# clearmatics/zecale

Measured on AMD Instinct MI355X. Metric: G1-MSM Mscalar/s (BW6_761, 2^20 terms per GPU), higher is better.
Workload: dtype u32; 1 GPU; BASELINE configs[1]: single MI355X G1_BW6_761 Pippenger MSM, 2^20 random scalars/points; terms_per_gpu=1048576, scalars=uniform in [0, r), Montgomery residues as libff holds them, parallelism=point-partitioned x1, RCCL all-gather of 288-byte partial sums

## Files before the change

include/zkhip.h:

```cpp
#ifndef ZKHIP_H
#define ZKHIP_H
#include <stddef.h>
#include <stdint.h>

#ifdef __cplusplus
extern "C" {
#endif

#define ZKHIP_OK 0
#define ZKHIP_ERR_ARG (-1)
#define ZKHIP_ERR_NO_DEVICE (-2)
#define ZKHIP_ERR_HIP (-3)
#define ZKHIP_ERR_STATE (-4)
#define ZKHIP_ERR_NO_TICKET (-5)

typedef struct zkhip_bases zkhip_bases;

int zkhip_init(int device);
int zkhip_set_device(int device);
int zkhip_get_device(void);
int zkhip_device_count(void);
int zkhip_device_memory(size_t* free_bytes, size_t* total_bytes);
void zkhip_shutdown(void);
const char* zkhip_strerror(int code);
// ... 198 lines not shown

typedef struct zkhip_keypair zkhip_keypair;
int zkhip_groth16_setup(const zkhip_r1cs_desc* cs, const uint64_t tau[6], const uint64_t alpha[6], const uint64_t beta[6],
                        const uint64_t delta[6], zkhip_keypair** out);
int zkhip_groth16_setup_ex(const zkhip_r1cs_desc* cs, const uint64_t tau[6], const uint64_t alpha[6], const uint64_t beta[6],
                           const uint64_t delta[6], size_t domain_size, zkhip_keypair** out);
int zkhip_groth16_setup_slice(const zkhip_r1cs_desc* cs, const uint64_t tau[6], const uint64_t alpha[6], const uint64_t beta[6],
                              const uint64_t delta[6], size_t domain_size, int parts, int part, const zkhip_key_opts* opts,
                              zkhip_crs** slice_out, size_t ranges[6], zkhip_keypair** vk_out);
int zkhip_keypair_crs_desc(const zkhip_keypair* kp, zkhip_crs_desc* out);
size_t zkhip_keypair_vk(const zkhip_keypair* kp, uint64_t alpha_g1[24], uint64_t beta_g2[24], uint64_t delta_g2[24],
                        const uint64_t** abc);
int zkhip_keypair_write(const zkhip_keypair* kp, const char* path);
int zkhip_keypair_read(const char* path, zkhip_keypair** out);
void zkhip_keypair_free(zkhip_keypair* kp);

float zkhip_last_accumulate_ms(void);
int zkhip_last_accumulate_entries(uint64_t* out);
int zkhip_last_accumulate_interval(float out_ms[2]);
int zkhip_reset_time_base(void);
int zkhip_measure_fq_mul_rate(double* fq_mul_per_s);
int zkhip_measure_ntt(unsigned log_d, int dir, int coset, int batch, int reps, double* ms_per_transform);
int zkhip_internal_field_selftest(int field, const uint32_t* limbs_in, size_t n, uint32_t* limbs_out);
int zkhip_internal_fq6_selftest(int op, const uint64_t* a, const uint64_t* b, size_t n, uint64_t* out);
int zkhip_internal_pairing_product(int route, const uint64_t* g1, const uint64_t* g2, size_t pairs_per_product, size_t count, uint64_t* out);
int zkhip_internal_tail_selftest(const uint64_t g1[24], const uint64_t g2[24], const uint64_t small_order_g1[24], int rounds);
typedef struct zkhip_witness_program {
  const uint8_t* code;
  const int32_t* a;
  const int32_t* b;
  size_t n_pos;
  const uint32_t* level_start;
  size_t n_levels;
  uint32_t chain_start;
  const int32_t* out_ref;
  size_t n_vars;
  const uint64_t* consts;
  size_t n_consts;
  size_t n_inputs;
} zkhip_witness_program;
int zkhip_internal_witness_run_program(const zkhip_witness_program* p, const uint64_t* inputs, size_t batches, int witnesses_per_workgroup,
                                       unsigned segment_chunks, uint64_t* z_out, uint32_t* flags_out);
int zkhip_internal_witness_run_program_wide(const zkhip_witness_program* p, const uint64_t* inputs, size_t batches, int witnesses_per_workgroup,
                                            unsigned segment_chunks, int waves, uint64_t* z_out, uint32_t* flags_out);
int zkhip_internal_pipeline_witness_sizing(size_t value_bytes, size_t mem_total, size_t wit_batch, int workers, size_t out[2]);
int zkhip_internal_witness_tape(zkhip_aggregator* a, zkhip_witness_program* out);
// ... 39 lines not shown
```

zecale_amd/csrc/msm.h:

```cpp
#pragma once
#include <hip/hip_runtime.h>
#include <stddef.h>
#include <stdint.h>

#include "../../include/zkhip.h"

namespace zkhip {

struct AffPacked;
struct EdwPacked;

#define MSM_MAX_AFF_LEVELS 4
#define MSM_MAX_JOBS 5
struct MsmJob {
  const AffPacked* bases;
  const uint8_t* inf_flags;
  const uint64_t* scalars;
  size_t n;
  int scalars_mode;
  size_t table_stride;
  size_t n_finite;
  const EdwPacked* edw = nullptr;
};
static inline size_t msm_job_terms(const MsmJob& j) { return (j.n_finite && j.n_finite < j.n) ? j.n_finite : j.n; }
// ... 1 lines not shown
#define ZK_PRIO_BOARD_WORDS (8 * 8 * 2 * 16 * 4 * 16)
struct MsmCtx {
  bool planned;
  int c, W, L, logL;
  int Wd;
  int merged;
  int K;
  uint16_t win_off[96];
  uint8_t win_bits[96];
  size_t B, max_n;
  size_t total_terms;
  int one_stream;
  uint32_t quad_below;
  uint32_t S, T, slot_stride;
  hipStream_t stream, stream2;
  hipEvent_t ev, ev2, ev_acc0, ev_acc1, ev_done;
  hipEvent_t acc_gate;
  uint32_t sort_LB, sort_NP, sort_bins, sort_tile;
  uint32_t* hist;
  uint2* pairs;
  size_t hist_len;
  uint32_t *counts, *offsets, *block_tot, *entries;
  uint32_t* goff;
  uint2* fix_list;
  uint2* fix_short;
  uint32_t *buckets, *segS[2], *segR, *sumR[2], *Rlevels, *colS[2], *hilo;
  uint64_t *win_abi, *win_host;
  int aff_levels;
  int aff_forced;
  uint32_t aff_m, aff_lanes;
  uint32_t *lcnt[MSM_MAX_AFF_LEVELS], *loff[MSM_MAX_AFF_LEVELS];
  AffPacked* pbuf[2];
  uint32_t* aff_scratch;
  size_t m_acc_max;
  float last_accumulate_ms;
  size_t last_hist_m;
  uint32_t acc_gen;
  float last_acc_begin_ms, last_acc_end_ms;
  uint64_t* dbg_times;
  uint32_t* prio_board;
  uint32_t prio_seq;
  uint32_t last_S, last_T;
  int last_tight;
  bool pending;
  size_t pending_n;
  bool win_edw;
  char errbuf[256];
};

void msm_force_aff_levels(int levels);
int msm_forced_aff_levels();
int msm_plan_init(MsmCtx* ctx, size_t max_n, int c, int merged, int K, size_t total_terms = 0, hipStream_t* adopt = nullptr);
hipEvent_t msm_time_base();
int msm_time_base_reset();
void msm_plan_free(MsmCtx* ctx);
int msm_bases_convert(const uint64_t* d_bases_abi, size_t n, AffPacked* d_out, uint8_t* d_inf_flags, char* errbuf, size_t errlen);
int msm_launch(MsmCtx* ctx, const AffPacked* d_bases, const uint8_t* d_inf_flags, const uint64_t* d_scalars, size_t n,
               int scalars_montgomery, size_t table_stride, const EdwPacked* edw = nullptr);
int msm_finish(MsmCtx* ctx, uint64_t out_jac[36]);
int msm_last_entries(MsmCtx* ctx, uint64_t* out);
int msm_launch_multi(MsmCtx* ctx, int K, const MsmJob* jobs);
int msm_finish_multi(MsmCtx* ctx, int K, uint64_t* out_jac);
static inline int msm_table_levels(int c, int naf = 0) { return naf ? 378 : (378 + c - 1) / c; }
int msm_table_build(AffPacked* d_table, uint8_t* d_tinf, size_t n, int c, int naf, char* errbuf, size_t errlen);
int msm_table_edw(const AffPacked* d_bases, const uint8_t* d_inf, size_t n, int c, EdwPacked** d_out, char* errbuf, size_t errlen);
static inline const EdwPacked* msm_edw_at(const EdwPacked* t, size_t i) {
  return t ? reinterpret_cast<const EdwPacked*>(reinterpret_cast<const char*>(t) + i * 288) : nullptr;
}

int msm_field_selftest(int field, const uint32_t* in_host, size_t n, uint32_t* out_host, char* errbuf, size_t errlen);
int msm_measure_fqmul_rate(double* fq_mul_per_s, char* errbuf, size_t errlen);

int fixed_base_mul(const uint64_t base_aff[24], const uint64_t* d_scalars, size_t n, int montgomery, uint64_t* d_out,
                   char* errbuf, size_t errlen);
// ... 3 lines not shown
```

zecale_amd/csrc/msm.hip:

```cpp
#include <hip/hip_runtime.h>
#include <stdint.h>
#include <stdio.h>
#include <stdlib.h>
#include <string.h>
#include <mutex>
#include <vector>

#include "ec_affine.cuh"
#include "ec_edw.cuh"
#include "host_field.hpp"
#include "msm.h"
#include "wait.h"


namespace zkhip {


__global__ void __launch_bounds__(256) k_bases_to_dev(const uint64_t* __restrict__ in, AffPacked* __restrict__ out,
                                                       uint8_t* __restrict__ inf_flags , size_t n) {
  size_t i = (size_t)blockIdx.x * blockDim.x + threadIdx.x;
  if (i >= n) return;
  uint64_t x[12], y[12];
  uint64_t nz = 0;
#pragma unroll
// ... 488 lines not shown
    const AffPacked* p = (dense ? bp.p[0] : base_of<NJ>(bp, b >> bshift)) + (e & 0x7fffffffu);
    const bool neg = (e >> 31) != 0;
    k++;
    if (dense && p->x[23] == ZK_AFF_INF_WORD) continue;
    if (madd_lds_regy(acc, xs, zz, zzz, ty, p, neg)) inf = fp_is_zero_2p(lds_ld(zz));
  }
  if (board_mine && (threadIdx.x & 63u) == 0) __hip_atomic_store(board_mine, (prio_tag << 16) | 0xffffu, __ATOMIC_RELAXED, __HIP_MEMORY_SCOPE_AGENT);
  if (!inf) {
    ZK_CLOSE_RUN(acc, xs, zz, zzz, ty);
  }
  if (dbg_times && (threadIdx.x & 63u) == 0) {
    const uint32_t wave = t >> 6;
    dbg_times[4 * wave] = dbg_t0; dbg_times[4 * wave + 1] = wall_clock64();
    dbg_times[4 * wave + 2] = __builtin_amdgcn_s_getreg((31 << 11) | 4);
    dbg_times[4 * wave + 3] = __builtin_amdgcn_s_getreg((31 << 11) | 20);
  }
}
template <int NJ>
__global__ void __launch_bounds__(256, 2) k_accumulate(ZK_ACC_PARAMS) {
  accumulate_impl<NJ, false>(bp, bshift, entries, offsets, counts, goff, nb, S_host, tight, T, slots, stride, fix_cnt, fix_short, fix_long,
                             dbg_times, prio_mode, prio_board, prio_tag);
}
__global__ void __launch_bounds__(256, 2) k_accumulate_edw(ZK_ACC_PARAMS) {
  accumulate_impl<1, true>(bp, bshift, entries, offsets, counts, goff, nb, S_host, tight, T, slots, stride, fix_cnt, fix_short, fix_long,
                           dbg_times, prio_mode, prio_board, prio_tag);
}

__global__ void __launch_bounds__(256) k_table_edw(const AffPacked* __restrict__ tab, const uint8_t* __restrict__ tinf, EdwPacked* __restrict__ out,
                                                   size_t total, uint32_t* __restrict__ bad) {
  const size_t i = (size_t)blockIdx.x * blockDim.x + threadIdx.x;
  if (i >= total) return;
  if (tinf[i]) {
    uint32_t* w = reinterpret_cast<uint32_t*>(out + i);
#pragma unroll
    for (int k = 0; k < 72; k++) w[k] = 0u;
    return;
  }
  const AffPacked* p = tab + i;
  if (!edw_from_affine(aff_ld_x(p), aff_ld_y(p, false), out + i)) atomicAdd(bad, 1u);
}

__global__ void __launch_bounds__(256) k_half_counts(const uint32_t* __restrict__ in_cnt, uint32_t* __restrict__ out_cnt, size_t nb) {
  size_t i = (size_t)blockIdx.x * blockDim.x + threadIdx.x;
  if (i < nb) out_cnt[i] = (in_cnt[i] + 1) >> 1;
}

struct LevelArgs {
  BasePtrs bp;
// ... 204 lines not shown
    for (uint32_t i = blockIdx.x * per + (QUAD ? threadIdx.x >> 2 : threadIdx.x); i < n; i += short_blocks * per) {
      const uint2 w = list_short[i];
      const XyzzRef dst = make_slot_ref(slots, stride, nb + w.x);
      for (uint32_t j = 1; j < w.y; j++) pt_add<QUAD, EDW>(dst, make_slot_ref(slots, stride, nb + w.x + j), q, sc);
    }
    return;
  }
  const uint32_t n = cnt[1], quad = threadIdx.x >> 2;
  for (uint32_t i = blockIdx.x - short_blocks; i < n; i += gridDim.x - short_blocks) {
    const uint2 w = list_long[i];
#pragma unroll 1
    for (uint32_t d = 1; d <= w.y - w.x; d <<= 1) {
      for (uint64_t t = (uint64_t)w.x + (uint64_t)quad * 2 * d; t + d <= w.y; t += (uint64_t)64 * 2 * d)
        pt_add<true, EDW>(make_slot_ref(slots, stride, nb + (uint32_t)t), make_slot_ref(slots, stride, nb + (uint32_t)t + d), q, sc);
      __threadfence_block();
      __syncthreads();
    }
  }
}
template <bool QUAD> __global__ void __launch_bounds__(256, 2) k_fixup_fold(ZK_FOLD_PARAMS) {
  fixup_fold_impl<QUAD, false>(cnt, list_short, list_long, short_blocks, nb, slots, stride);
}
template <bool QUAD> __global__ void __launch_bounds__(256, 2) k_fixup_fold_edw(ZK_FOLD_PARAMS) {
  fixup_fold_impl<QUAD, true>(cnt, list_short, list_long, short_blocks, nb, slots, stride);
}

#define ZK_FIXUP_PARAMS                                                                                                             \
  const uint32_t* __restrict__ offsets, const uint32_t* __restrict__ counts, const uint32_t* __restrict__ goff, uint32_t nb, uint32_t S_host, \
      int tight, uint32_t T, uint32_t* __restrict__ slots, uint32_t stride, uint32_t wf
template <bool EDW>
__device__ __forceinline__ void fixup_impl(ZK_FIXUP_PARAMS) {
  __shared__ uint32_t lds_zz[27 * ZK_LDS_STRIDE], lds_zzz[27 * ZK_LDS_STRIDE], lds_x[24 * ZK_LDS_STRIDE];
  uint32_t t = blockIdx.x * blockDim.x + threadIdx.x;
  const uint32_t M = offsets[nb - 1] + counts[nb - 1];
  const uint32_t A = slice_weight(goff[nb], T, S_host, tight);
  if (t >= T) return;
  uint32_t b0_, b1_;
  const uint32_t pos0 = slice_pos(goff, offsets, counts, nb, M, (uint64_t)t * A, &b0_, wf);
  if (pos0 >= M) return;
  const uint32_t pos1 = slice_pos(goff, offsets, counts, nb, M, (uint64_t)(t + 1) * A, &b1_, wf);
  uint32_t b = bucket_of(offsets, nb, pos1 - 1);
  uint32_t bend = offsets[b] + counts[b];
  if (bend <= pos1 || offsets[b] < pos0) return;
  const XyzzRef dst = make_slot_ref(slots, stride, b), pl = make_slot_ref(slots, stride, nb + T + t), pf = make_slot_ref(slots, stride, nb + t + 1);
  const bool l_inf = mem_is_inf(pl), f_inf = mem_is_inf(pf);
  if (l_inf || f_inf) {
    if (l_inf && f_inf) mem_set_inf(dst);
    else mem_copy(dst, l_inf ? pf : pl);
    return;
  }
  uint32_t* zz = lds_zz + threadIdx.x;
  uint32_t* zzz = lds_zzz + threadIdx.x;
  uint32_t* xs = lds_x + threadIdx.x;
  lds_st_packed(xs, mem_ld(pl, CX));
  Fq ty = mem_ld(pl, CY);
  lds_st(zz, mem_ld(pl, CZZ));
  lds_st(zzz, mem_ld(pl, CZZZ));
  if (pt_add_lds<EDW>(dst, xs, zz, zzz, ty, pf)) { mem_set_inf(dst); return; }
  mem_st(dst, CX, lds_ld_packed(xs)); mem_st(dst, CY, ty); mem_st(dst, CZZ, lds_ld(zz)); mem_st(dst, CZZZ, lds_ld(zzz));
}
__global__ void __launch_bounds__(256, 2) k_fixup(ZK_FIXUP_PARAMS) { fixup_impl<false>(offsets, counts, goff, nb, S_host, tight, T, slots, stride, wf); }
__global__ void __launch_bounds__(256, 2) k_fixup_edw(ZK_FIXUP_PARAMS) { fixup_impl<true>(offsets, counts, goff, nb, S_host, tight, T, slots, stride, wf); }

#define ZK_SEG_PARAMS uint32_t* __restrict__ in, size_t n_in, uint32_t in_stride, int L, int o, uint32_t* __restrict__ outS, uint32_t* __restrict__ outR
template <bool QUAD, bool EDW>
__device__ __forceinline__ void seg_impl(ZK_SEG_PARAMS) {
  ADD_SCRATCH_DECL(QUAD || EDW);
  size_t n_out = n_in / L;
  size_t gt = (size_t)blockIdx.x * blockDim.x + threadIdx.x, t = QUAD ? gt >> 2 : gt;
  const uint32_t q = (uint32_t)(gt & 3);
  if (t >= n_out) return;
  XyzzRef run = make_ref(outS, (uint32_t)n_out, (uint32_t)t), acc = make_ref(outR, (uint32_t)n_out, (uint32_t)t);
  pt_set_inf<QUAD>(run, q);
  pt_set_inf<QUAD>(acc, q);
  for (int u = L - 1; u >= 0; u--) {
    XyzzRef it = make_ref(in, in_stride, (uint32_t)(t * L + u));
    pt_add<QUAD, EDW>(run, it, q, sc);
    if (u + o > 0) pt_add<QUAD, EDW>(acc, run, q, sc);
  }
}
template <bool QUAD> __global__ void __launch_bounds__(256, 2) k_seg(ZK_SEG_PARAMS) { seg_impl<QUAD, false>(in, n_in, in_stride, L, o, outS, outR); }
template <bool QUAD> __global__ void __launch_bounds__(256, 2) k_seg_edw(ZK_SEG_PARAMS) { seg_impl<QUAD, true>(in, n_in, in_stride, L, o, outS, outR); }

#define ZK_SUM_PARAMS                                                                                       \
  uint32_t* __restrict__ in, size_t n_in, uint32_t in_stride, int L, uint32_t row_len, uint32_t* __restrict__ out, \
// ... 403 lines not shown
    const char* e = getenv("ZKHIP_SLICE_TARGET");
    v = e ? (size_t)atoi(e) : 80;
    if (v < 8 || v > 4096) v = 80;
  }
  return v;
}

static int env_int(const char* name, int dflt, int lo, int hi) {
  const char* e = getenv(name);
  if (!e) return dflt;
  int v = atoi(e);
  return (v < lo || v > hi) ? dflt : v;
}
static size_t level_bound(size_t m, size_t nb) { return (m + (m < nb ? m : nb)) / 2; }
static int g_aff_forced = -2;
void msm_force_aff_levels(int levels) { g_aff_forced = levels < -1 ? -1 : (levels > MSM_MAX_AFF_LEVELS ? MSM_MAX_AFF_LEVELS : levels); }
int msm_forced_aff_levels() { return g_aff_forced == -2 ? env_int("ZKHIP_AFF_LEVELS", -1, 0, MSM_MAX_AFF_LEVELS) : g_aff_forced; }
static int choose_aff_levels(size_t m_entries, size_t nb) {
  (void)m_entries; (void)nb;
  int forced = msm_forced_aff_levels();
  return forced >= 0 ? forced : 0;
}

static hipEvent_t g_time_base[64];
static bool g_time_base_made[64];
static uint32_t g_time_base_gen[64];
static std::mutex g_time_base_mu;
static hipEvent_t time_base_locked(int dev, bool renew) {
  if (!g_time_base_made[dev] && hipEventCreate(&g_time_base[dev]) != hipSuccess) return nullptr;
  if (!g_time_base_made[dev] || renew) {
    if (hipEventRecord(g_time_base[dev], 0) != hipSuccess || hipEventSynchronize(g_time_base[dev]) != hipSuccess) {
      if (!g_time_base_made[dev]) (void)hipEventDestroy(g_time_base[dev]);
      return nullptr;
    }
    g_time_base_made[dev] = true;
  }
  return g_time_base[dev];
}
hipEvent_t msm_time_base() {
  int dev = 0;
  if (hipGetDevice(&dev) != hipSuccess || dev < 0 || dev >= 64) dev = 0;
  std::lock_guard<std::mutex> lk(g_time_base_mu);
  return time_base_locked(dev, false);
}
int msm_time_base_reset() {
  int dev = 0;
// ... 84 lines not shown
  HIP_TRY(hipEventCreateWithFlags(&ctx->ev_done, hipEventBlockingSync | hipEventDisableTiming));
  if ((size_t)ctx->Wd * max_n >= ((size_t)1 << 31)) return ZKHIP_ERR_ARG;
  if ((size_t)ctx->Wd * total_terms >= ((size_t)1 << 32)) return ZKHIP_ERR_ARG;
  {
    uint32_t LB = (uint32_t)(c - 1 < 10 ? c - 1 : 10);
    const size_t want_parts = (size_t)env_int("ZKHIP_SORT_PARTS", 1024, 64, 8192);
    while (LB > 6 && (nb >> LB) < want_parts && (ctx->B >> (LB - 1)) * (merged ? 1 : (size_t)ctx->Wd) <= 4096) LB--;
    ctx->sort_LB = LB;
    ctx->sort_NP = (uint32_t)(ctx->B >> LB);
    ctx->sort_bins = merged ? ctx->sort_NP : ctx->sort_NP * (uint32_t)ctx->Wd;
    if ((size_t)ctx->sort_bins * 8 > 60 * 1024) return ZKHIP_ERR_ARG;
    uint32_t tile = (uint32_t)env_int("ZKHIP_SORT_TILE", 1024, 256, 16384) & ~255u;
    while ((max_n + tile - 1) / tile > 1024) tile *= 2;
    ctx->sort_tile = tile;
    const size_t nbx = (max_n + tile - 1) / tile;
    ctx->hist_len = (nb >> LB) * (nbx ? nbx : 1) + 1;
  }
  HIP_TRY(hipMalloc(&ctx->hist, ctx->hist_len * 4));
  HIP_TRY(hipMalloc(&ctx->pairs, ((size_t)ctx->Wd * total_terms + 1) * sizeof(uint2)));
  HIP_TRY(hipMalloc(&ctx->counts, nb * 4));
  HIP_TRY(hipMalloc(&ctx->offsets, nb * 4));
  HIP_TRY(hipMalloc(&ctx->goff, (nb + 1) * 4));
  if ((size_t)ctx->Wd * total_terms * ZK_W_NEXT >= ((size_t)1 << 32)) return ZKHIP_ERR_ARG;
  HIP_TRY(hipMalloc(&ctx->block_tot, ((nb > ctx->hist_len ? nb : ctx->hist_len) / 1024 + 2) * 4));
  HIP_TRY(hipMalloc(&ctx->entries, ((size_t)ctx->Wd * total_terms + 1) * 4));
  {
    size_t m = (size_t)ctx->Wd * total_terms;
    ctx->aff_levels = choose_aff_levels(m, nb);
    ctx->aff_forced = msm_forced_aff_levels();
    ctx->aff_m = (uint32_t)env_int("ZKHIP_AFF_M", 64, 4, 512);
    ctx->aff_lanes = 1u << 18;
    const size_t m_cap = (size_t)ctx->aff_m * 3 / 2;
    while ((size_t)ctx->aff_lanes * m_cap * 108 >= ((size_t)1 << 32)) ctx->aff_lanes >>= 1;
    size_t bound[MSM_MAX_AFF_LEVELS + 1];
    bound[0] = m;
    for (int l = 0; l < ctx->aff_levels; l++) {
      bound[l + 1] = level_bound(bound[l], nb);
      HIP_TRY(hipMalloc(&ctx->lcnt[l], nb * 4));
      HIP_TRY(hipMalloc(&ctx->loff[l], nb * 4));
    }
    if (ctx->aff_levels > 0) {
      HIP_TRY(hipMalloc(&ctx->pbuf[0], (bound[1] + 1) * sizeof(AffPacked)));
      if (ctx->aff_levels > 1) HIP_TRY(hipMalloc(&ctx->pbuf[1], (bound[2] + 1) * sizeof(AffPacked)));
      size_t lanes = (bound[1] + ctx->aff_m - 1) / ctx->aff_m;
      if (lanes < ctx->aff_lanes) ctx->aff_lanes = (uint32_t)((lanes + 255) & ~(size_t)255);
      HIP_TRY(hipMalloc(&ctx->aff_scratch, (size_t)ctx->aff_lanes * m_cap * 108));
    }
// ... 20 lines not shown
  ctx->prio_seq = 0;
  HIP_TRY(hipMalloc(&ctx->fix_list, ((size_t)ctx->T / 5 + 2) * sizeof(uint2)));
  HIP_TRY(hipMalloc(&ctx->fix_short, ((size_t)ctx->T / 2 + 2) * sizeof(uint2)));
  HIP_TRY(hipMalloc(&ctx->segS[0], (nb / 2 + 1) * 108 * 4));
  HIP_TRY(hipMalloc(&ctx->segS[1], (nb / 2 + 1) * 108 * 4));
  HIP_TRY(hipMalloc(&ctx->segR, (nb / 2 + 64 * (size_t)ctx->W) * 108 * 4));
  HIP_TRY(hipMalloc(&ctx->sumR[0], (nb / ctx->L / ctx->L + 4 * ctx->W + 1) * 108 * 4));
  HIP_TRY(hipMalloc(&ctx->sumR[1], (nb / ctx->L / ctx->L + 4 * ctx->W + 1) * 108 * 4));
  HIP_TRY(hipMalloc(&ctx->Rlevels, (size_t)32 * 2 * ctx->W * 108 * 4));
  HIP_TRY(hipMalloc(&ctx->colS[0], (nb / 2 + 1) * 108 * 4));
  HIP_TRY(hipMalloc(&ctx->colS[1], (nb / 2 + 1) * 108 * 4));
  HIP_TRY(hipMalloc(&ctx->hilo, ((size_t)2 * ctx->W * ((size_t)1 << ((c - 1 + 1) / 2)) + 8) * 108 * 4));
  HIP_TRY(hipMalloc(&ctx->win_abi, (size_t)ctx->W * 48 * 8 * 2));
  HIP_TRY(hipHostMalloc(&ctx->win_host, (size_t)ctx->W * 48 * 8 * 2));
  ctx->planned = true;
  return ZKHIP_OK;
}

void msm_plan_free(MsmCtx* ctx) {
  void* ptrs[] = {ctx->hist, ctx->pairs, ctx->counts, ctx->offsets, ctx->block_tot, ctx->entries, ctx->buckets,
                  ctx->segS[0], ctx->segS[1], ctx->segR, ctx->sumR[0], ctx->sumR[1], ctx->Rlevels, ctx->win_abi,
                  ctx->colS[0], ctx->colS[1], ctx->hilo, ctx->pbuf[0], ctx->pbuf[1], ctx->aff_scratch,
                  ctx->lcnt[0], ctx->lcnt[1], ctx->lcnt[2], ctx->lcnt[3], ctx->loff[0], ctx->loff[1], ctx->loff[2], ctx->loff[3],
                  ctx->fix_list, ctx->fix_short, ctx->dbg_times, ctx->goff, ctx->prio_board};
  for (void* p : ptrs) if (p) (void)hipFree(p);
  if (ctx->win_host) (void)hipHostFree(ctx->win_host);
  if (ctx->stream) (void)hipStreamDestroy(ctx->stream);
  if (ctx->stream2) (void)hipStreamDestroy(ctx->stream2);
  if (ctx->ev) (void)hipEventDestroy(ctx->ev);
  if (ctx->ev2) (void)hipEventDestroy(ctx->ev2);
  if (ctx->ev_acc0) (void)hipEventDestroy(ctx->ev_acc0);
  if (ctx->ev_acc1) (void)hipEventDestroy(ctx->ev_acc1);
  if (ctx->ev_done) (void)hipEventDestroy(ctx->ev_done);
  memset(ctx, 0, sizeof *ctx);
}

int msm_bases_convert(const uint64_t* d_bases_abi, size_t n, AffPacked* d_out, uint8_t* d_inf_flags, char* errbuf, size_t errlen) {
  hipLaunchKernelGGL(k_bases_to_dev, dim3(nblk(n, 256)), dim3(256), 0, 0, d_bases_abi, d_out, d_inf_flags, n);
  hipError_t e = hipGetLastError();
  if (e == hipSuccess) e = hipDeviceSynchronize();
  if (e != hipSuccess) {
    if (errbuf) snprintf(errbuf, errlen, "msm_bases_convert: %s", hipGetErrorString(e));
    return ZKHIP_ERR_HIP;
  }
  return ZKHIP_OK;
}

// ... 82 lines not shown
    const size_t lanes_tot = (m_out + la.m - 1) / la.m;
    for (size_t lane0 = 0; lane0 < lanes_tot; lane0 += ctx->aff_lanes) {
      const size_t ln = lanes_tot - lane0 < ctx->aff_lanes ? lanes_tot - lane0 : ctx->aff_lanes;
      la.lane0 = (uint32_t)lane0; la.lanes = ctx->aff_lanes;
      const dim3 grid(nblk(ln, 256));
      if (l == 0) {
        if (ctx->K == 1) hipLaunchKernelGGL((k_affine_level<1, true>), grid, dim3(256), 0, st, la);
        else hipLaunchKernelGGL((k_affine_level<MSM_MAX_JOBS, true>), grid, dim3(256), 0, st, la);
      } else {
        hipLaunchKernelGGL((k_affine_level<1, false>), grid, dim3(256), 0, st, la);
      }
    }
    cur_off = ctx->loff[l]; cur_cnt = ctx->lcnt[l]; m_cur = m_out;
  }
  const bool dense = ctx->aff_levels > 0;
  if (dense) bp.p[0] = ctx->pbuf[(ctx->aff_levels - 1) & 1];
  {
    const unsigned gb = nblk(nb + 1, 1024);
    hipLaunchKernelGGL(k_slice_weights, dim3(nblk(nb + 1, 256)), dim3(256), 0, st, cur_cnt, ctx->goff, nb, wf);
    hipLaunchKernelGGL(k_scan_local, dim3(gb), dim3(256), 0, st, ctx->goff, ctx->goff, ctx->block_tot, nb + 1);
    hipLaunchKernelGGL(k_scan_tot, dim3(1), dim3(1024), 0, st, ctx->block_tot, (size_t)gb);
    hipLaunchKernelGGL(k_scan_add, dim3(gb), dim3(256), 0, st, ctx->goff, ctx->block_tot, nb + 1);
  }
  HIP_TRY(hipMemsetAsync(ctx->block_tot, 0, 8, st));
  uint32_t S_run, T_run;
  {
    const size_t lanes = 131072, m = m_cur;
    size_t fills = (m + lanes * slice_target() - 1) / (lanes * slice_target());
    if (fills < 1) fills = 1;
    size_t S = (m + lanes * fills - 1) / (lanes * fills);
    if (S < 16) S = 16;
    if (ctx->one_stream) S *= (size_t)env_int("ZKHIP_STREAM_SLICE_MULT", 2, 1, 16);
    {
      size_t n_jobs = 0;
      for (int k = 0; k < K; k++) n_jobs += jobs[k].n ? 1 : 0;
      const size_t live_buckets = merged ? B * (n_jobs ? n_jobs : 1) : nb, avg = m / (live_buckets ? live_buckets : 1);
      if (S < (avg + 1) / 2) S = (avg + 1) / 2;
    }
    while ((m + S - 1) / S > ctx->T) S++;
    S_run = (uint32_t)S; T_run = (uint32_t)((m + S - 1) / S);
  }
  const int tight = (ctx->one_stream || dense) ? 0 : env_int("ZKHIP_TIGHT_SLICES", 1, 0, 1);
#if ZK_SLOTS_AOS
  {
    static const int clear_mode = env_int("ZKHIP_SLOTS_CLEAR", 0, 0, 1);
    if (clear_mode == 1) HIP_TRY(hipMemsetAsync(ctx->buckets, 0, (size_t)ctx->slot_stride * ZK_SLOT_WORDS * 4, st));
    else hipLaunchKernelGGL(k_slots_clear_zz, dim3(nblk((size_t)ctx->slot_stride * 27, 256)), dim3(256), 0, st, ctx->buckets, ctx->slot_stride);
  }
#else
  HIP_TRY(hipMemsetAsync(ctx->buckets + (size_t)CZZ * 27 * ctx->slot_stride, 0, (size_t)ctx->slot_stride * 27 * 4, st));
#endif
  if (ctx->dbg_times) HIP_TRY(hipMemsetAsync(ctx->dbg_times, 0, ((size_t)ctx->T / 64 + 8) * 32, st));
  if (ctx->acc_gate) HIP_TRY(hipStreamWaitEvent(st, ctx->acc_gate, 0));
  if (ctx->aff_levels == 0) HIP_TRY(hipEventRecord(ctx->ev_acc0, st));
  const uint32_t* acc_entries = dense ? nullptr : ctx->entries;
  static const int acc_prio = env_int("ZKHIP_ACC_PRIO", 1, 0, 2);
  const uint32_t prio_tag = (++ctx->prio_seq & 0x7fffu) + 1u;
  if (edw)
    hipLaunchKernelGGL(k_accumulate_edw, dim3(nblk(T_run, 256)), dim3(256), 0, st, bp, bshift, acc_entries, cur_off, cur_cnt, ctx->goff,
                       (uint32_t)nb, S_run, tight, T_run, ctx->buckets, ctx->slot_stride, ctx->block_tot + 0, ctx->fix_short, ctx->fix_list, ctx->dbg_times, acc_prio, (acc_prio == 1 && !ctx->one_stream) ? ctx->prio_board : (uint32_t*)nullptr, prio_tag);
  else if (ctx->K == 1 || dense)
    hipLaunchKernelGGL(k_accumulate<1>, dim3(nblk(T_run, 256)), dim3(256), 0, st, bp, bshift, acc_entries, cur_off, cur_cnt, ctx->goff,
                       (uint32_t)nb, S_run, tight, T_run, ctx->buckets, ctx->slot_stride, ctx->block_tot + 0, ctx->fix_short, ctx->fix_list, ctx->dbg_times, acc_prio, (acc_prio == 1 && !ctx->one_stream) ? ctx->prio_board : (uint32_t*)nullptr, prio_tag);
  else
    hipLaunchKernelGGL(k_accumulate<MSM_MAX_JOBS>, dim3(nblk(T_run, 256)), dim3(256), 0, st, bp, bshift, acc_entries, cur_off,
                       cur_cnt, ctx->goff, (uint32_t)nb, S_run, tight, T_run, ctx->buckets, ctx->slot_stride, ctx->block_tot + 0, ctx->fix_short, ctx->fix_list, ctx->dbg_times, acc_prio, (acc_prio == 1 && !ctx->one_stream) ? ctx->prio_board : (uint32_t*)nullptr, prio_tag);
  HIP_TRY(hipEventRecord(ctx->ev_acc1, st));
  ctx->last_S = S_run; ctx->last_T = T_run; ctx->last_tight = tight;
  if (T_run > 2) {
    const bool fold_quads = T_run < (1u << 18) && ctx->quad_below > 1024;
    const uint32_t per = fold_quads ? 64u : 256u;
    uint32_t sblocks = nblk((size_t)T_run / 2 + 1, per);
    if (sblocks > 1024) sblocks = 1024;
    auto fold = fold_quads ? (edw ? k_fixup_fold_edw<true> : k_fixup_fold<true>) : (edw ? k_fixup_fold_edw<false> : k_fixup_fold<false>);
    hipLaunchKernelGGL(fold, dim3(sblocks + 512), dim3(256), 0, st, ctx->block_tot, ctx->fix_short, ctx->fix_list, sblocks, (uint32_t)nb, ctx->buckets,
                       ctx->slot_stride);
  }
  hipLaunchKernelGGL(edw ? k_fixup_edw : k_fixup, dim3(nblk(T_run, 256)), dim3(256), 0, st, cur_off, cur_cnt, ctx->goff, (uint32_t)nb, S_run, tight,
                     T_run, ctx->buckets, ctx->slot_stride, wf);
  HIP_TRY(hipGetLastError());

  const size_t QUAD_BELOW = ctx->quad_below;
  hipStream_t st2 = ctx->one_stream ? ctx->stream : ctx->stream2;
  const int lo_bits = (c - 1 + 1) / 2, hi_bits = (c - 1) - lo_bits;
  const uint32_t Rr = 1u << lo_bits, Hh = 1u << hi_bits, Nn = Rr > Hh ? Rr : Hh;
  auto launch_sum = [&](hipStream_t s_, uint32_t* in, size_t n_in, uint32_t in_stride, int L, uint32_t row_len, uint32_t* out) {
    size_t n_out = n_in / L;
    const int in_slots = (in == ctx->buckets) ? 1 : 0;
    if (n_out >= QUAD_BELOW) hipLaunchKernelGGL(edw ? k_sum_lds_edw : k_sum_lds, dim3(nblk(n_out, 256)), dim3(256), 0, s_, in, n_in, in_stride, L, row_len, out, in_slots);
    else hipLaunchKernelGGL(edw ? k_sum_edw<true> : k_sum<true>, dim3(nblk(n_out * 4, 256)), dim3(256), 0, s_, in, n_in, in_stride, L, row_len, out, in_slots);
  };
  HIP_TRY(hipEventRecord(ctx->ev, st));
  HIP_TRY(hipStreamWaitEvent(st2, ctx->ev, 0));
  uint32_t *rows = nullptr, *cols = nullptr;
  {
    uint32_t* in = ctx->buckets; uint32_t in_stride = ctx->slot_stride; size_t n_in = nb; uint32_t left = Rr; int pp = 0;
    if (left == 1) rows = in;
    auto tree_fan_in = [&](size_t n_in_, uint32_t left_) {
      int L = ctx->L;
      if (n_in_ / (size_t)L < QUAD_BELOW) L = 2;
      while ((uint32_t)L > left_) L >>= 1;
      return L;
// ... 262 lines not shown
```

zecale_amd/csrc/zkhip_api.hip:

```cpp
#include <math.h>
#include <hip/hip_runtime.h>
#include <stdio.h>
#include <string.h>
#include <atomic>
#include <memory>
#include <mutex>

#include "ec.cuh"
#include "host_field.hpp"
#include "domain.hpp"
#include "msm.h"
#include "wait.h"
#include "ntt.h"
#include "qap.h"
#include "pairing_host.hpp"
#include "pairing.h"
#include "witness.h"
#include <chrono>
#include <condition_variable>
#include <deque>
#include <functional>
#include <future>
#include <thread>
#include <vector>
// ... 2227 lines not shown
  std::lock_guard<std::mutex> lk(st->mu);
  return st->last_accumulate_ms;
}
int zkhip_msm_stream_last_accumulate_interval(zkhip_msm_stream* st, float out_ms[2]) {
  if (!st || !out_ms) return fail(ZKHIP_ERR_ARG, "null pointer");
  std::lock_guard<std::mutex> lk(st->mu);
  out_ms[0] = st->last_interval[0]; out_ms[1] = st->last_interval[1];
  return ZKHIP_OK;
}

int zkhip_measure_fq_mul_rate(double* fq_mul_per_s) {
  BIND_CUR();
  if (!fq_mul_per_s) return fail(ZKHIP_ERR_ARG, "null pointer");
  std::lock_guard<std::mutex> lk(g.dev[cur_dev()].mu);
  return msm_measure_fqmul_rate(fq_mul_per_s, t_err, sizeof t_err);
}

int zkhip_measure_ntt(unsigned log_d, int dir, int coset, int batch, int reps, double* ms_per_transform) {
  BIND_CUR();
  if (!ms_per_transform) return fail(ZKHIP_ERR_ARG, "null pointer");
  return ntt_measure((int)log_d, dir, coset, batch, reps, ms_per_transform, t_err, sizeof t_err);
}

int zkhip_internal_field_selftest(int field, const uint32_t* limbs_in, size_t n, uint32_t* limbs_out) {
  BIND_CUR();
  if ((field != 0 && field != 1) || (n && (!limbs_in || !limbs_out)) || n > (1u << 20)) return fail(ZKHIP_ERR_ARG, "field 0 (Fq) or 1 (Fr), at most 2^20 cases");
  std::lock_guard<std::mutex> lk(g.dev[cur_dev()].mu);
  return msm_field_selftest(field, limbs_in, n, limbs_out, t_err, sizeof t_err);
}

int zkhip_internal_tail_selftest(const uint64_t g1[24], const uint64_t g2[24], const uint64_t small[24], int rounds) {
  using namespace host;
  if (!g1 || !g2 || !small || rounds < 0 || rounds > 100000) return fail(ZKHIP_ERR_ARG, "tail selftest: arguments");
  auto aff = [](const uint64_t* p) { return HJac::from_affine(HFq::from_limbs(p), HFq::from_limbs(p + 12)); };
  auto same = [](const HJac& a, const HJac& b) {
    if (a.is_inf() || b.is_inf()) return a.is_inf() && b.is_inf();
    HFq ax, ay, bx, by;
    a.to_affine(ax, ay); b.to_affine(bx, by);
    uint64_t l[4][12];
    ax.to_limbs(l[0]); ay.to_limbs(l[1]); bx.to_limbs(l[2]); by.to_limbs(l[3]);
    return !memcmp(l[0], l[2], 96) && !memcmp(l[1], l[3], 96);
  };
  uint64_t r_m[6], s_m[6];
  HFr::from_u64(0x1234567u).to_limbs(r_m);
  (HFr::from_u64(0x89abcdefu) * HFr::from_u64(0xfedcba98u) * HFr::from_u64(0x76543211u)).to_limbs(s_m);
  for (int i = 0; i < rounds; i++) {
// ... 52 lines not shown
```

zecale_amd/zkhip.py:

```python
import ctypes
import os

import numpy as np

_HERE = os.path.dirname(os.path.abspath(__file__))
LIB_PATH = os.environ.get("ZKHIP_LIB") or os.path.join(_HERE, "libzkhip.so")

EXPORTS = [
    "zkhip_init", "zkhip_set_device", "zkhip_get_device", "zkhip_device_count", "zkhip_fr_random", "zkhip_shutdown", "zkhip_strerror", "zkhip_last_error", "zkhip_set_msm_window", "zkhip_set_affine_levels",
    "zkhip_bases_upload", "zkhip_bases_upload_dev", "zkhip_bases_len", "zkhip_bases_free",
    "zkhip_bases_precompute", "zkhip_bases_table_window", "zkhip_set_crs_precompute", "zkhip_crs_table_window", "zkhip_set_batch_msms",
    "zkhip_msm", "zkhip_msm_dev", "zkhip_msm_raw", "zkhip_msm_submit", "zkhip_msm_collect",
    "zkhip_device_alloc", "zkhip_device_free", "zkhip_device_copy_in", "zkhip_last_accumulate_ms", "zkhip_last_accumulate_entries", "zkhip_prover_last_accumulate_entries",
    "zkhip_prover_set_streaming", "zkhip_set_table_naf", "zkhip_set_table_model", "zkhip_bases_table_model", "zkhip_fixed_base_mul", "zkhip_fixed_base_mul_dev", "zkhip_ntt", "zkhip_ntt_dev",
    "zkhip_r1cs_upload", "zkhip_r1cs_upload_ex", "zkhip_r1cs_set_domain", "zkhip_r1cs_free", "zkhip_r1cs_log_domain", "zkhip_r1cs_domain_size",
    "zkhip_domain_size", "zkhip_step_domain_size", "zkhip_domain_is_valid", "zkhip_groth16_setup_ex", "zkhip_dispatcher_outstanding", "zkhip_r1cs_is_satisfied", "zkhip_qap_h",
    "zkhip_crs_upload", "zkhip_crs_free", "zkhip_groth16_prove", "zkhip_last_prove_timings", "zkhip_groth16_verify",
    "zkhip_crs_upload_slice", "zkhip_groth16_prove_partial", "zkhip_groth16_finish",
    "zkhip_bls12_377_groth16_verify", "zkhip_aggregator_new", "zkhip_aggregator_free", "zkhip_aggregator_num_constraints",
    "zkhip_aggregator_num_variables", "zkhip_aggregator_num_primary_inputs", "zkhip_aggregator_get_r1cs",
    "zkhip_aggregator_witness", "zkhip_aggregator_witness_gpu", "zkhip_gpu_witness_new", "zkhip_gpu_witness_new_batched", "zkhip_gpu_witness_run", "zkhip_gpu_witness_run_batched", "zkhip_gpu_witness_free",
    "zkhip_gpu_witness_stats", "zkhip_prover_prove_dev", "zkhip_aggregator_check_inputs", "zkhip_aggregator_vk_hash", "zkhip_aggregator_num_proofs", "zkhip_aggregator_inputs_per_proof",
    "zkhip_prover_new", "zkhip_prover_create_streams", "zkhip_prover_prove", "zkhip_prover_timings", "zkhip_prover_free", "zkhip_prover_last_accumulate_ms",
    "zkhip_aggregator_pipeline_new", "zkhip_aggregator_pipeline_new_ex", "zkhip_crs_device", "zkhip_aggregator_pipeline_submit", "zkhip_aggregator_pipeline_wait", "zkhip_aggregator_pipeline_free",
    "zkhip_groth16_setup", "zkhip_groth16_setup_slice", "zkhip_keypair_crs_desc", "zkhip_keypair_vk", "zkhip_keypair_free", "zkhip_keypair_write", "zkhip_keypair_read",
    "zkhip_jac_to_affine", "zkhip_jac_add", "zkhip_to_canonical",
    "zkhip_last_accumulate_interval", "zkhip_crs_upload_ex", "zkhip_crs_upload_slice_ex", "zkhip_bases_precompute_ex", "zkhip_crs_table_kind", "zkhip_crs_finite_terms",
    "zkhip_bases_set_window", "zkhip_reset_time_base", "zkhip_measure_fq_mul_rate", "zkhip_internal_field_selftest", "zkhip_internal_tail_selftest", "zkhip_internal_pipeline_witness_sizing", "zkhip_internal_witness_run_program", "zkhip_internal_witness_run_program_wide", "zkhip_internal_witness_tape", "zkhip_internal_gpu_witness_run", "zkhip_internal_gpu_witness_run_wide", "zkhip_gpu_witness_set_waves", "zkhip_gpu_witness_plan", "zkhip_gpu_witness_last_ms", "zkhip_device_memory", "zkhip_last_prove_split", "zkhip_set_prove_split", "zkhip_host_alloc", "zkhip_host_free",
    "zkhip_msm_stream_new", "zkhip_msm_stream_submit", "zkhip_msm_stream_submit_host", "zkhip_msm_stream_collect", "zkhip_msm_stream_last_accumulate_ms",
    "zkhip_msm_stream_last_accumulate_interval", "zkhip_msm_stream_free", "zkhip_prover_new_slice", "zkhip_prover_prove_partial",
    "zkhip_dispatcher_new", "zkhip_dispatcher_size", "zkhip_dispatcher_submit", "zkhip_dispatcher_wait", "zkhip_dispatcher_stats", "zkhip_dispatcher_free",
    "zkhip_multi_prover_new", "zkhip_multi_prover_size", "zkhip_multi_prover_prove", "zkhip_multi_prover_timings", "zkhip_multi_prover_free",
    "zkhip_aggregator_app_new", "zkhip_aggregator_app_free", "zkhip_aggregator_app_num_constants", "zkhip_aggregator_app_constants", "zkhip_aggregator_app_mask",
    "zkhip_aggregator_witness_app", "zkhip_groth16_prove_app", "zkhip_prover_prove_app", "zkhip_prover_prove_app_dev", "zkhip_gpu_witness_run_batched_app",
    "zkhip_aggregator_pipeline_register_app", "zkhip_aggregator_pipeline_app_hits", "zkhip_dispatcher_register_app", "zkhip_device_copy_out", "zkhip_measure_ntt", "zkhip_key_partition", "zkhip_prover_timings_chained",
    "zkhip_verifier_new", "zkhip_verifier_num_inputs", "zkhip_verifier_verify_batch", "zkhip_verifier_free", "zkhip_internal_fq6_selftest", "zkhip_internal_pairing_product",
]


class ZkhipError(RuntimeError):

    def __init__(self, msg, code=None):
        super().__init__(msg)
        self.code = code


c_u64p_t = ctypes.POINTER(ctypes.c_uint64)


class R1csDesc(ctypes.Structure):
    _fields_ = [("n_constraints", ctypes.c_size_t), ("n_vars", ctypes.c_size_t), ("n_primary", ctypes.c_size_t)] + [
        (f"{m}_{k}", ctypes.c_void_p) for m in "abc" for k in ("row_ptr", "col", "val")]


class KeyOpts(ctypes.Structure):
    _fields_ = [("precompute", ctypes.c_int), ("table_naf", ctypes.c_int), ("window", ctypes.c_int), ("batch_msms", ctypes.c_int)]


def key_opts(precompute=None, table_naf=None, window=0, batch_msms=None):
# ... 1203 lines not shown
def jac_to_affine(jac):
    j = np.ascontiguousarray(jac, dtype=np.uint64)
    out = np.zeros(24, dtype=np.uint64)
    _check(load().zkhip_jac_to_affine(_p(j), _p(out)))
    return out


def jac_add(a, b):
    out = np.zeros(36, dtype=np.uint64)
    _check(load().zkhip_jac_add(_p(np.ascontiguousarray(a, dtype=np.uint64)), _p(np.ascontiguousarray(b, dtype=np.uint64)), _p(out)))
    return out


def last_accumulate_ms():
    return float(load().zkhip_last_accumulate_ms())


def last_accumulate_entries():
    out = ctypes.c_uint64(0)
    _check(load().zkhip_last_accumulate_entries(ctypes.byref(out)))
    return int(out.value)


def field_selftest(field, limbs_in):
    nl = 27 if field == 0 else 14
    x = np.ascontiguousarray(limbs_in, dtype=np.uint32).reshape(-1, 4, nl)
    out = np.zeros((x.shape[0], 3, nl), dtype=np.uint32)
    lib = load()
    lib.zkhip_internal_field_selftest.argtypes = [ctypes.c_int, ctypes.c_void_p, ctypes.c_size_t, ctypes.c_void_p]
    _check(lib.zkhip_internal_field_selftest(int(field), x.ctypes.data, x.shape[0], out.ctypes.data))
    return out


def witness_run_program(prog, inputs, wpg=4, segment=2048, waves=1):
    arrs = dict(code=np.ascontiguousarray(prog["code"], dtype=np.uint8), a=np.ascontiguousarray(prog["a"], dtype=np.int32), b=np.ascontiguousarray(prog["b"], dtype=np.int32),
                level_start=np.ascontiguousarray(prog["level_start"], dtype=np.uint32), out_ref=np.ascontiguousarray(prog["out_ref"], dtype=np.int32),
                consts=np.ascontiguousarray(prog["consts"], dtype=np.uint64).reshape(-1, 6))
    n = arrs["code"].size
    assert arrs["a"].size == n and arrs["b"].size == n and arrs["level_start"].size >= 1
    x = np.ascontiguousarray(inputs, dtype=np.uint64).reshape(-1, int(prog["n_inputs"]), 6) if int(prog["n_inputs"]) else np.zeros((len(inputs), 0, 6), dtype=np.uint64)
    ptr = lambda k: arrs[k].ctypes.data if arrs[k].size else None
    wp = WitnessProgram(ptr("code"), ptr("a"), ptr("b"), n, arrs["level_start"].ctypes.data, arrs["level_start"].size - 1, int(prog["chain_start"]),
                        ptr("out_ref"), arrs["out_ref"].size, ptr("consts"), arrs["consts"].shape[0], int(prog["n_inputs"]))
    batches = x.shape[0]
    z = np.zeros((batches, arrs["out_ref"].size, 6), dtype=np.uint64)
    flags = np.zeros(max(batches, 1), dtype=np.uint32)
# ... 36 lines not shown
```

Baseline: 103.4 Mscalar/s.

## Add lockstep Edwards bucket accumulation with count-sorted bucket ordering

Adds a counting sort of buckets by their entry count (a two-pass histogram plus scan) so that an alternative Edwards accumulate kernel can assign one bucket per thread. Neighbouring lanes then hold buckets of similar size and run nearly the same number of loop iterations. The new path is enabled by default. It runs only when no bucket exceeds 128 entries and enough buckets are live; in that case the existing segmented accumulate, fold and fixup kernels exit early. This is meant to remove the segmentation and fixup overhead and the wave divergence of the general path. In exchange it adds several extra sort and scan kernel launches and an order array, and kernels are still launched that may immediately return.

```diff
diff --git a/include/zkhip.h b/include/zkhip.h
--- a/include/zkhip.h
+++ b/include/zkhip.h
@@ -244,6 +244,8 @@
 int zkhip_measure_fq_mul_rate(double* fq_mul_per_s);
 int zkhip_measure_ntt(unsigned log_d, int dir, int coset, int batch, int reps, double* ms_per_transform);
 int zkhip_internal_field_selftest(int field, const uint32_t* limbs_in, size_t n, uint32_t* limbs_out);
+int zkhip_internal_set_lockstep(int mode, int min_buckets);
+int zkhip_internal_last_acc_path(int* out);
 int zkhip_internal_fq6_selftest(int op, const uint64_t* a, const uint64_t* b, size_t n, uint64_t* out);
 int zkhip_internal_pairing_product(int route, const uint64_t* g1, const uint64_t* g2, size_t pairs_per_product, size_t count, uint64_t* out);
 int zkhip_internal_tail_selftest(const uint64_t g1[24], const uint64_t g2[24], const uint64_t small_order_g1[24], int rounds);
diff --git a/zecale_amd/csrc/msm.h b/zecale_amd/csrc/msm.h
--- a/zecale_amd/csrc/msm.h
+++ b/zecale_amd/csrc/msm.h
@@ -47,6 +47,8 @@
   size_t hist_len;
   uint32_t *counts, *offsets, *block_tot, *entries;
   uint32_t* goff;
+  uint32_t *order, *ord_hist;
+  uint32_t lock_min_live;
   uint2* fix_list;
   uint2* fix_short;
   uint32_t *buckets, *segS[2], *segR, *sumR[2], *Rlevels, *colS[2], *hilo;
@@ -75,6 +77,8 @@
 
 void msm_force_aff_levels(int levels);
 int msm_forced_aff_levels();
+void msm_force_lockstep(int mode, int min_buckets);
+int msm_last_acc_path(MsmCtx* ctx, int* out);
 int msm_plan_init(MsmCtx* ctx, size_t max_n, int c, int merged, int K, size_t total_terms = 0, hipStream_t* adopt = nullptr);
 hipEvent_t msm_time_base();
 int msm_time_base_reset();
diff --git a/zecale_amd/csrc/msm.hip b/zecale_amd/csrc/msm.hip
--- a/zecale_amd/csrc/msm.hip
+++ b/zecale_amd/csrc/msm.hip
@@ -534,8 +534,67 @@
                              dbg_times, prio_mode, prio_board, prio_tag);
 }
 __global__ void __launch_bounds__(256, 2) k_accumulate_edw(ZK_ACC_PARAMS) {
+  if (fix_cnt[2] == 1u) return;
   accumulate_impl<1, true>(bp, bshift, entries, offsets, counts, goff, nb, S_host, tight, T, slots, stride, fix_cnt, fix_short, fix_long,
                            dbg_times, prio_mode, prio_board, prio_tag);
+}
+
+#define ZK_LOCK_CAP 128u
+#define ZK_LOCK_KEYS (ZK_LOCK_CAP + 2u)
+__device__ __forceinline__ uint32_t lock_key(uint32_t cnt) { return cnt > ZK_LOCK_CAP ? 0u : ZK_LOCK_CAP + 1u - cnt; }
+template <int PASS>
+__global__ void __launch_bounds__(256) k_bucket_order(const uint32_t* __restrict__ counts, uint32_t nb, uint32_t* __restrict__ ohist,
+                                                       uint32_t* __restrict__ order, uint32_t* __restrict__ lock_ok, uint32_t min_live, int enable) {
+  __shared__ uint32_t s_k[ZK_LOCK_KEYS];
+  const uint32_t tid = threadIdx.x, nblocks = gridDim.x;
+  for (uint32_t j = tid; j < ZK_LOCK_KEYS; j += 256) s_k[j] = PASS == 0 ? 0u : ohist[(size_t)j * nblocks + blockIdx.x];
+  __syncthreads();
+#pragma unroll
+  for (int k = 0; k < 4; k++) {
+    const uint32_t b = blockIdx.x * 1024u + (uint32_t)k * 256u + tid;
+    if (b < nb) {
+      const uint32_t pos = atomicAdd(&s_k[lock_key(counts[b])], 1u);
+      if (PASS == 1 && pos < nb) order[pos] = b;
+    }
+  }
+  if (PASS == 0) {
+    __syncthreads();
+    for (uint32_t j = tid; j < ZK_LOCK_KEYS; j += 256) ohist[(size_t)j * nblocks + blockIdx.x] = s_k[j];
+  } else if (blockIdx.x == 0 && tid == 0) {
+    const uint32_t over = ohist[nblocks], live = ohist[(size_t)(ZK_LOCK_CAP + 1u) * nblocks];
+    *lock_ok = (enable && over == 0u && live >= min_live) ? 1u : 0u;
+  }
+}
+
+__global__ void __launch_bounds__(256, 2) k_accumulate_edw_lock(const EdwPacked* __restrict__ etab, const uint32_t* __restrict__ entries,
+                                                                 const uint32_t* __restrict__ offsets, const uint32_t* __restrict__ counts,
+                                                                 const uint32_t* __restrict__ order, uint32_t nb, uint32_t* __restrict__ slots,
+                                                                 uint32_t stride, const uint32_t* __restrict__ lock_ok) {
+  if (*lock_ok == 0u) return;
+  const uint32_t t = blockIdx.x * blockDim.x + threadIdx.x;
+  __shared__ uint32_t lds_zz[27 * ZK_LDS_STRIDE], lds_zzz[27 * ZK_LDS_STRIDE], lds_x[24 * ZK_LDS_STRIDE];
+  uint32_t* zz = lds_zz + threadIdx.x;
+  uint32_t* zzz = lds_zzz + threadIdx.x;
+  uint32_t* xs = lds_x + threadIdx.x;
+  const uint32_t b = t < nb ? order[t] : 0u;
+  const uint32_t cnt = t < nb ? counts[b] : 0u;
+  const uint32_t trip = (uint32_t)__builtin_amdgcn_readfirstlane((int)cnt);
+  if (trip == 0u) return;
+  const uint32_t off = offsets[b];
+  Fq ty;
+  edw_set_identity(xs, zz, zzz, ty);
+  uint32_t e_next = cnt ? entries[off] : 0u;
+  for (uint32_t j = 0; j < trip; j++) {
+    if (j < cnt) {
+      const uint32_t e = e_next;
+      if (j + 1 < cnt) e_next = entries[off + j + 1];
+      edw_madd_lds_regy(xs, zz, zzz, ty, etab + (e & 0x7fffffffu), (e >> 31) != 0);
+    }
+  }
+  if (cnt) {
+    XyzzRef acc = make_slot_ref(slots, stride, b);
+    ZK_CLOSE_RUN(acc, xs, zz, zzz, ty);
+  }
 }
 
 __global__ void __launch_bounds__(256) k_table_edw(const AffPacked* __restrict__ tab, const uint8_t* __restrict__ tinf, EdwPacked* __restrict__ out,
@@ -786,6 +845,7 @@
   fixup_fold_impl<QUAD, false>(cnt, list_short, list_long, short_blocks, nb, slots, stride);
 }
 template <bool QUAD> __global__ void __launch_bounds__(256, 2) k_fixup_fold_edw(ZK_FOLD_PARAMS) {
+  if (cnt[2] == 1u) return;
   fixup_fold_impl<QUAD, true>(cnt, list_short, list_long, short_blocks, nb, slots, stride);
 }
 
@@ -824,7 +884,10 @@
   mem_st(dst, CX, lds_ld_packed(xs)); mem_st(dst, CY, ty); mem_st(dst, CZZ, lds_ld(zz)); mem_st(dst, CZZZ, lds_ld(zzz));
 }
 __global__ void __launch_bounds__(256, 2) k_fixup(ZK_FIXUP_PARAMS) { fixup_impl<false>(offsets, counts, goff, nb, S_host, tight, T, slots, stride, wf); }
-__global__ void __launch_bounds__(256, 2) k_fixup_edw(ZK_FIXUP_PARAMS) { fixup_impl<true>(offsets, counts, goff, nb, S_host, tight, T, slots, stride, wf); }
+__global__ void __launch_bounds__(256, 2) k_fixup_edw(ZK_FIXUP_PARAMS, const uint32_t* __restrict__ lock_ok) {
+  if (*lock_ok == 1u) return;
+  fixup_impl<true>(offsets, counts, goff, nb, S_host, tight, T, slots, stride, wf);
+}
 
 #define ZK_SEG_PARAMS uint32_t* __restrict__ in, size_t n_in, uint32_t in_stride, int L, int o, uint32_t* __restrict__ outS, uint32_t* __restrict__ outR
 template <bool QUAD, bool EDW>
@@ -1274,6 +1337,23 @@
   return forced >= 0 ? forced : 0;
 }
 
+#define ZK_LOCKSTEP_DEFAULT 1
+static int g_lock_forced = -1, g_lock_min_live = -1;
+void msm_force_lockstep(int mode, int min_buckets) { g_lock_forced = mode < 0 ? -1 : (mode ? 1 : 0); g_lock_min_live = min_buckets < 0 ? -1 : min_buckets; }
+static int lockstep_mode() {
+  static const int env_mode = env_int("ZKHIP_LOCKSTEP", ZK_LOCKSTEP_DEFAULT, 0, 1);
+  return g_lock_forced >= 0 ? g_lock_forced : env_mode;
+}
+int msm_last_acc_path(MsmCtx* ctx, int* out) {
+  *out = -1;
+  if (!ctx->planned || !ctx->win_edw || !ctx->order) return ZKHIP_OK;
+  uint32_t v = 0;
+  HIP_TRY(hipDeviceSynchronize());
+  HIP_TRY(hipMemcpy(&v, ctx->block_tot + 2, 4, hipMemcpyDeviceToHost));
+  *out = (int)v;
+  return ZKHIP_OK;
+}
+
 static hipEvent_t g_time_base[64];
 static bool g_time_base_made[64];
 static uint32_t g_time_base_gen[64];
@@ -1404,7 +1484,20 @@
   HIP_TRY(hipMalloc(&ctx->offsets, nb * 4));
   HIP_TRY(hipMalloc(&ctx->goff, (nb + 1) * 4));
   if ((size_t)ctx->Wd * total_terms * ZK_W_NEXT >= ((size_t)1 << 32)) return ZKHIP_ERR_ARG;
-  HIP_TRY(hipMalloc(&ctx->block_tot, ((nb > ctx->hist_len ? nb : ctx->hist_len) / 1024 + 2) * 4));
+  const size_t ord_m = (size_t)ZK_LOCK_KEYS * nblk(nb, 1024);
+  {
+    size_t scan_m = nb > ctx->hist_len ? nb : ctx->hist_len;
+    if (ord_m > scan_m) scan_m = ord_m;
+    HIP_TRY(hipMalloc(&ctx->block_tot, (scan_m / 1024 + 4) * 4));
+  }
+  if (merged == 1 && K == 1) {
+    HIP_TRY(hipMalloc(&ctx->order, nb * 4));
+    HIP_TRY(hipMalloc(&ctx->ord_hist, ord_m * 4));
+    int dev = 0, cus = 0;
+    HIP_TRY(hipGetDevice(&dev));
+    HIP_TRY(hipDeviceGetAttribute(&cus, hipDeviceAttributeMultiprocessorCount, dev));
+    ctx->lock_min_live = 64u * 2u * 4u * (uint32_t)(cus > 0 ? cus : 256);
+  }
   HIP_TRY(hipMalloc(&ctx->entries, ((size_t)ctx->Wd * total_terms + 1) * 4));
   {
     size_t m = (size_t)ctx->Wd * total_terms;
@@ -1471,7 +1564,7 @@
                   ctx->segS[0], ctx->segS[1], ctx->segR, ctx->sumR[0], ctx->sumR[1], ctx->Rlevels, ctx->win_abi,
                   ctx->colS[0], ctx->colS[1], ctx->hilo, ctx->pbuf[0], ctx->pbuf[1], ctx->aff_scratch,
                   ctx->lcnt[0], ctx->lcnt[1], ctx->lcnt[2], ctx->lcnt[3], ctx->loff[0], ctx->loff[1], ctx->loff[2], ctx->loff[3],
-                  ctx->fix_list, ctx->fix_short, ctx->dbg_times, ctx->goff, ctx->prio_board};
+                  ctx->fix_list, ctx->fix_short, ctx->dbg_times, ctx->goff, ctx->prio_board, ctx->order, ctx->ord_hist};
   for (void* p : ptrs) if (p) (void)hipFree(p);
   if (ctx->win_host) (void)hipHostFree(ctx->win_host);
   if (ctx->stream) (void)hipStreamDestroy(ctx->stream);
@@ -1600,6 +1693,16 @@
     hipLaunchKernelGGL(k_scan_tot, dim3(1), dim3(1024), 0, st, ctx->block_tot, (size_t)gb);
     hipLaunchKernelGGL(k_scan_add, dim3(gb), dim3(256), 0, st, ctx->goff, ctx->block_tot, nb + 1);
   }
+  if (edw) {
+    const unsigned ob = nblk(nb, 1024), os = nblk((size_t)ZK_LOCK_KEYS * ob, 1024);
+    const int lock_on = lockstep_mode();
+    const uint32_t min_live = g_lock_min_live >= 0 ? (uint32_t)g_lock_min_live : ctx->lock_min_live;
+    hipLaunchKernelGGL(k_bucket_order<0>, dim3(ob), dim3(256), 0, st, cur_cnt, (uint32_t)nb, ctx->ord_hist, ctx->order, ctx->block_tot + 2, min_live, lock_on);
+    hipLaunchKernelGGL(k_scan_local, dim3(os), dim3(256), 0, st, ctx->ord_hist, ctx->ord_hist, ctx->block_tot, (size_t)ZK_LOCK_KEYS * ob);
+    hipLaunchKernelGGL(k_scan_tot, dim3(1), dim3(1024), 0, st, ctx->block_tot, (size_t)os);
+    hipLaunchKernelGGL(k_scan_add, dim3(os), dim3(256), 0, st, ctx->ord_hist, ctx->block_tot, (size_t)ZK_LOCK_KEYS * ob);
+    hipLaunchKernelGGL(k_bucket_order<1>, dim3(ob), dim3(256), 0, st, cur_cnt, (uint32_t)nb, ctx->ord_hist, ctx->order, ctx->block_tot + 2, min_live, lock_on);
+  }
   HIP_TRY(hipMemsetAsync(ctx->block_tot, 0, 8, st));
   uint32_t S_run, T_run;
   {
@@ -1634,10 +1737,12 @@
   const uint32_t* acc_entries = dense ? nullptr : ctx->entries;
   static const int acc_prio = env_int("ZKHIP_ACC_PRIO", 1, 0, 2);
   const uint32_t prio_tag = (++ctx->prio_seq & 0x7fffu) + 1u;
-  if (edw)
+  if (edw) {
+    hipLaunchKernelGGL(k_accumulate_edw_lock, dim3(nblk(nb, 256)), dim3(256), 0, st, jobs[0].edw, ctx->entries, cur_off, cur_cnt, ctx->order, (uint32_t)nb,
+                       ctx->buckets, ctx->slot_stride, ctx->block_tot + 2);
     hipLaunchKernelGGL(k_accumulate_edw, dim3(nblk(T_run, 256)), dim3(256), 0, st, bp, bshift, acc_entries, cur_off, cur_cnt, ctx->goff,
                        (uint32_t)nb, S_run, tight, T_run, ctx->buckets, ctx->slot_stride, ctx->block_tot + 0, ctx->fix_short, ctx->fix_list, ctx->dbg_times, acc_prio, (acc_prio == 1 && !ctx->one_stream) ? ctx->prio_board : (uint32_t*)nullptr, prio_tag);
-  else if (ctx->K == 1 || dense)
+  } else if (ctx->K == 1 || dense)
     hipLaunchKernelGGL(k_accumulate<1>, dim3(nblk(T_run, 256)), dim3(256), 0, st, bp, bshift, acc_entries, cur_off, cur_cnt, ctx->goff,
                        (uint32_t)nb, S_run, tight, T_run, ctx->buckets, ctx->slot_stride, ctx->block_tot + 0, ctx->fix_short, ctx->fix_list, ctx->dbg_times, acc_prio, (acc_prio == 1 && !ctx->one_stream) ? ctx->prio_board : (uint32_t*)nullptr, prio_tag);
   else
@@ -1654,8 +1759,12 @@
     hipLaunchKernelGGL(fold, dim3(sblocks + 512), dim3(256), 0, st, ctx->block_tot, ctx->fix_short, ctx->fix_list, sblocks, (uint32_t)nb, ctx->buckets,
                        ctx->slot_stride);
   }
-  hipLaunchKernelGGL(edw ? k_fixup_edw : k_fixup, dim3(nblk(T_run, 256)), dim3(256), 0, st, cur_off, cur_cnt, ctx->goff, (uint32_t)nb, S_run, tight,
-                     T_run, ctx->buckets, ctx->slot_stride, wf);
+  if (edw)
+    hipLaunchKernelGGL(k_fixup_edw, dim3(nblk(T_run, 256)), dim3(256), 0, st, cur_off, cur_cnt, ctx->goff, (uint32_t)nb, S_run, tight, T_run, ctx->buckets,
+                       ctx->slot_stride, wf, ctx->block_tot + 2);
+  else
+    hipLaunchKernelGGL(k_fixup, dim3(nblk(T_run, 256)), dim3(256), 0, st, cur_off, cur_cnt, ctx->goff, (uint32_t)nb, S_run, tight, T_run, ctx->buckets,
+                       ctx->slot_stride, wf);
   HIP_TRY(hipGetLastError());
 
   const size_t QUAD_BELOW = ctx->quad_below;
diff --git a/zecale_amd/csrc/zkhip_api.hip b/zecale_amd/csrc/zkhip_api.hip
--- a/zecale_amd/csrc/zkhip_api.hip
+++ b/zecale_amd/csrc/zkhip_api.hip
@@ -2273,6 +2273,23 @@
   return ntt_measure((int)log_d, dir, coset, batch, reps, ms_per_transform, t_err, sizeof t_err);
 }
 
+int zkhip_internal_set_lockstep(int mode, int min_buckets) {
+  msm_force_lockstep(mode, min_buckets);
+  return ZKHIP_OK;
+}
+int zkhip_internal_last_acc_path(int* out) {
+  if (!out) return fail(ZKHIP_ERR_ARG, "null argument");
+  *out = -1;
+  const int dev = t_prove_dev >= 0 ? t_prove_dev : cur_dev();
+  if (dev < 0) return ZKHIP_OK;
+  { int rc_ = bind_dev(dev); if (rc_ != ZKHIP_OK) return rc_; }
+  std::lock_guard<std::mutex> lk(g.dev[dev].mu);
+  MsmCtx* cx = g.dev[dev].ps.last_acc_ctx;
+  if (!cx) return ZKHIP_OK;
+  const int rc = msm_last_acc_path(cx, out);
+  return rc == ZKHIP_OK ? rc : ctx_fail(rc, cx);
+}
+
 int zkhip_internal_field_selftest(int field, const uint32_t* limbs_in, size_t n, uint32_t* limbs_out) {
   BIND_CUR();
   if ((field != 0 && field != 1) || (n && (!limbs_in || !limbs_out)) || n > (1u << 20)) return fail(ZKHIP_ERR_ARG, "field 0 (Fq) or 1 (Fr), at most 2^20 cases");
diff --git a/zecale_amd/zkhip.py b/zecale_amd/zkhip.py
--- a/zecale_amd/zkhip.py
+++ b/zecale_amd/zkhip.py
@@ -34,7 +34,7 @@
     "zkhip_aggregator_app_new", "zkhip_aggregator_app_free", "zkhip_aggregator_app_num_constants", "zkhip_aggregator_app_constants", "zkhip_aggregator_app_mask",
     "zkhip_aggregator_witness_app", "zkhip_groth16_prove_app", "zkhip_prover_prove_app", "zkhip_prover_prove_app_dev", "zkhip_gpu_witness_run_batched_app",
     "zkhip_aggregator_pipeline_register_app", "zkhip_aggregator_pipeline_app_hits", "zkhip_dispatcher_register_app", "zkhip_device_copy_out", "zkhip_measure_ntt", "zkhip_key_partition", "zkhip_prover_timings_chained",
-    "zkhip_verifier_new", "zkhip_verifier_num_inputs", "zkhip_verifier_verify_batch", "zkhip_verifier_free", "zkhip_internal_fq6_selftest", "zkhip_internal_pairing_product",
+    "zkhip_verifier_new", "zkhip_verifier_num_inputs", "zkhip_verifier_verify_batch", "zkhip_verifier_free", "zkhip_internal_fq6_selftest", "zkhip_internal_pairing_product", "zkhip_internal_set_lockstep", "zkhip_internal_last_acc_path",
 ]
 
 
@@ -1284,6 +1284,16 @@
     return int(out.value)
 
 
+def set_lockstep(mode, min_buckets=-1):
+    _check(load().zkhip_internal_set_lockstep(int(mode), int(min_buckets)))
+
+
+def last_acc_path():
+    out = ctypes.c_int(-1)
+    _check(load().zkhip_internal_last_acc_path(ctypes.byref(out)))
+    return int(out.value)
+
+
 def field_selftest(field, limbs_in):
     nl = 27 if field == 0 else 14
     x = np.ascontiguousarray(limbs_in, dtype=np.uint32).reshape(-1, 4, nl)
```

New measurement: 108.9 Mscalar/s (median of 6 runs). 1.05x the previous value.
